# crisprVerse/screenCounter

Hardware: NVIDIA B200
Metric: reads/sec (higher is better)
Workload: dtype u32

## Files before the change

### screencounter_b200/csrc/jit.cpp

```cpp
#include "jit.hpp"

#include <dlfcn.h>
#include <sys/stat.h>
#include <sys/types.h>
#include <unistd.h>

#include <algorithm>
#include <cerrno>
#include <chrono>
#include <cstdio>

#include <cstdlib>
#include <cstring>
#include <map>
#include <mutex>
#include <sstream>
#include <vector>

#include "common.hpp"
#include "layout.hpp"

namespace scg {

namespace {
// ... 263 lines not shown
        if (rc != 0) {
            size_t log_size = 0;
            n.GetProgramLogSize(p, &log_size);
            std::string log(log_size, '\0');
            if (log_size) n.GetProgramLog(p, &log[0]);
            n.DestroyProgram(&p);
            return remember(std::string("nvrtcCompileProgram: ") + n.GetErrorString(rc) + "\n" + log);
        }
        size_t cubin_size = 0;
        n.GetCUBINSize(p, &cubin_size);
        cubin.resize(cubin_size);
        rc = n.GetCUBIN(p, cubin.data());
        n.DestroyProgram(&p);
        if (rc != 0 || cubin_size == 0) return remember("nvrtcGetCUBIN failed");
        if (!path.empty()) disk_store(path, disk_key, cubin);
    }
    if (const char* dump = std::getenv("SCG_DUMP_CUBIN")) {
        const std::string out = std::string(dump) + "/" + prog.name + ".cubin";
        if (FILE* f = std::fopen(out.c_str(), "wb")) {
            std::fwrite(cubin.data(), 1, cubin.size(), f);
            std::fclose(f);
        }
    }
    cudaError_t st = cudaLibraryLoadData(&entry.library, cubin.data(), nullptr, nullptr, 0, nullptr, nullptr, 0);
    if (st != cudaSuccess) {
        cudaGetLastError();
        return remember(std::string("cudaLibraryLoadData: ") + cudaGetErrorString(st));
    }
    for (const std::string& name : prog.kernels) {
        cudaKernel_t k = nullptr;
        st = cudaLibraryGetKernel(&k, entry.library, name.c_str());
        if (st != cudaSuccess) {
            cudaGetLastError();
            return remember("cudaLibraryGetKernel(" + name + "): " + cudaGetErrorString(st));
        }
        entry.kernels.push_back(k);
    }
    entry.build_s = wall_s() - t0;
    g_jit_seconds += entry.build_s;
    auto& slot = g_cache[key];
    slot = entry;
    return &slot;
}

double jit_seconds_total() { return g_jit_seconds; }

int jit_env_int(const char* name, int fallback, int lo, int hi) {
    const char* v = std::getenv(name);
    if (!v || !*v) return fallback;
    int x = std::atoi(v);
    return x < lo ? lo : (x > hi ? hi : x);
}

cudaKernel_t specialised_single_kernel(const SpecSingleConfig& cfg, int device, std::string* why, cudaKernel_t* slow) {
    auto fail = [&](const std::string& msg) -> cudaKernel_t {
        if (why) *why = msg;
        return nullptr;
    };
    if (cfg.W > (cfg.ulen > 0 ? 10 : 6)) {
        return fail(cfg.ulen > 0 ? "reads longer than 320 bases use the generic kernel" : "reads longer than 192 bases use the generic kernel");
    }
    if (cfg.T > 128) return fail("templates longer than 128 bases use the generic kernel");
    if (cfg.cb > 3) return fail("mismatch budgets above 7 use the generic kernel");
    if (cfg.keylen > 32) return fail("variable regions longer than 32 bases use the generic kernel");

    const int min_blocks = jit_env_int("SCG_SPEC_MIN_BLOCKS", cfg.ulen > 0 ? (cfg.W <= 3 ? 8 : (cfg.W <= 6 ? 6 : 4)) : 4, 1, 16);
    const int stages = jit_env_int("SCG_SPEC_STAGES", 2, 1, 8);
    const int group = jit_env_int("SCG_SPEC_GROUP", (cfg.ulen > 0 && cfg.W >= 6) ? 1 : 2, 1, 8);
    const int samples = jit_env_int("SCG_SPEC_SAMPLES", 8, 1, 32);

    std::string seed_list = "{ ";
    for (size_t k = 0; k < cfg.seed_masks.size(); ++k) seed_list += (k ? ", " : "") + std::to_string(cfg.seed_masks[k]) + "u";
    if (cfg.seed_masks.empty()) seed_list += "0u";
    seed_list += " }";
    std::ostringstream src;
    const int nb_max = (32 * cfg.W - cfg.T + 1 + 31) / 32;
    const int nb = std::max(1, std::min(cfg.nb, nb_max));
    src << "#define SPEC_CUSTOM 1\n"
        << "#define SPEC_T " << cfg.T << "\n"
        << "#define SPEC_FBASES \"" << cfg.fbases << "\"\n"
        << "#define SPEC_RBASES \"" << cfg.rbases << "\"\n"
        << "#define SPEC_FWD " << cfg.fwd << "\n"
        << "#define SPEC_REV " << cfg.rev << "\n"
        << "#define SPEC_W " << cfg.W << "\n"
        << "#define SPEC_NB " << nb << "\n"
        << "#define SPEC_CB " << cfg.cb << "\n"
        << "#define SPEC_MM " << cfg.mm << "\n"
        << "#define SPEC_MAXMM " << cfg.maxmm << "\n"
        << "#define SPEC_USE_FIRST " << cfg.use_first << "\n"
        << "#define SPEC_FSTART " << cfg.fstart << "\n"
        << "#define SPEC_RSTART " << cfg.rstart << "\n"
        << "#define SPEC_KEYLEN " << cfg.keylen << "\n"
        << "#define SPEC_NSEEDS " << cfg.seed_masks.size() << "\n"
        << "#define SPEC_SEEDMASKS " << seed_list << "\n"
        << "#define SPEC_DUP_FIRST " << cfg.dup_first << "\n"
        << "#define SPEC_NAME spec_single_kernel\n"
        << "#define SPEC_MIN_BLOCKS " << min_blocks << "\n"
        << "#define SPEC_STAGES " << stages << "\n"
        << "#define SPEC_ULEN " << cfg.ulen << "\n"
        << "#define SPEC_NAME_U spec_single_kernel_u\n"
        << "#define SPEC_NAME_SLOW spec_single_kernel_slow\n"
        << "#define SPEC_GROUP " << group << "\n"
        << "#define SPEC_SAMPLES " << samples << "\n"
        << "#define SPEC_INFO " << cfg.info << "\n"
        << "#define SPEC_JOINT " << cfg.joint << "\n"
        << "#define SPEC_HAS_INDEX " << cfg.has_index << "\n"
        << "#define SPEC_IBUCKETS " << cfg.ibuckets << "\n"
        << "#define SPEC_RAGGED " << cfg.ragged << "\n"
        << "#define SPEC_HIST " << cfg.hist << "\n"
        << "#define SPEC_PRED " << cfg.pred << "\n"
        << "#define SPEC_UWARP " << jit_env_int("SCG_SPEC_UWARP", 0, 0, 1) << "\n"
        << "#define SPEC_SKIP_GENERAL " << (cfg.ulen > 0 ? 1 : 0) << "\n"
        << "#include \"spec_single.cuh\"\n";
    JitProgram prog;
    prog.name = "spec_single_jit.cu";
    prog.text = src.str();
    if (cfg.ulen > 0) {
        prog.kernels = { "spec_single_kernel_u", "spec_single_kernel_slow" };
    } else {
        prog.kernels = { "spec_single_kernel" };
    }
    const JitModule* mod = jit_module(prog, device, why);
    if (!mod) return nullptr;
    if (slow) *slow = cfg.ulen > 0 ? mod->kernels[1] : nullptr;
    return mod->kernels[0];
}

}
```

### screencounter_b200/csrc/jit.hpp

```cpp
#pragma once

#include <cuda_runtime.h>

#include <string>
#include <vector>

#include "handlers_params.hpp"
#include "template_spec.hpp"

namespace scg {

struct SpecSingleConfig {
    std::string fbases, rbases;
    int T = 0, fwd = 0, rev = 0;
    int W = 0;
    int nb = 1;
    int cb = 0, mm = 0, maxmm = 0, use_first = 1;
    int fstart = 0, rstart = 0, keylen = 0;
    std::vector<uint32_t> seed_masks;
    int dup_first = 0;
    int ulen = 0;
    int info = 1;
    int joint = 0;
    int has_index = 1;
    int ibuckets = 0;
    int ragged = 0;
    int pred = 0;
    int hist = 0;
    std::string key() const;
};

struct JitProgram {
    std::string name;
    std::string text;
    std::vector<std::string> kernels;
};
struct JitModule {
    cudaLibrary_t library = nullptr;
    std::vector<cudaKernel_t> kernels;
    std::string problem;
    bool from_disk = false;
    double build_s = 0;
};
const JitModule* jit_module(const JitProgram& prog, int device, std::string* why);
double jit_seconds_total();
int jit_env_int(const char* name, int fallback, int lo, int hi);

cudaKernel_t specialised_single_kernel(const SpecSingleConfig& cfg, int device, std::string* why, cudaKernel_t* slow = nullptr);

int specialised_blocks_per_sm(cudaKernel_t kernel);

std::string jit_status();

}
```

### screencounter_b200/csrc/runners_single.cu

```cuda
#include <algorithm>
#include <chrono>
#include <cstring>
#include <exception>
#include <thread>

#include "api_common.hpp"
#include "hostpool.hpp"
#include "handlers.cuh"
#include "jit.hpp"
#include "launchers.hpp"
#include "matchers.hpp"

namespace scg {

std::string& creation_error() {
    static thread_local std::string msg;
    return msg;
}

static double now_s() {
    return std::chrono::duration<double>(std::chrono::steady_clock::now().time_since_epoch()).count();
}

Pool::Pool(const char* const* p, int n) {
// ... 284 lines not shown
    if (lib.KW != 1 || lib.nseeds < 1 || lib.nseeds > 4 || lib.cand_rows.empty()) return;
    for (int s = 0; s < lib.nseeds; ++s) {
        if (lib.seed_masks[s] == 0) {
            cfg.seed_masks.clear();
            return;
        }
        cfg.seed_masks.push_back(lib.seed_masks[s]);
    }
}

void launch_single(Context& ctx, const ReadsDev& reads, const SingleMatcher& m, int32_t* d_counts, int32_t* d_index, uint32_t* d_info,
                   cudaStream_t stream) {
    if (reads.n <= 0) return;
    const SingleParams& P = m.params;
    const long long ntiles = (reads.n + TILE - 1) / TILE;
    const int grid = ctx.grid_for(ntiles);

    SpecSingleConfig cfg;
    cfg.fbases = m.tmpl.fwd_seq;
    cfg.rbases = m.tmpl.rev ? m.tmpl.rev_seq : std::string(m.tmpl.length, '-');
    cfg.T = m.tmpl.length;
    cfg.fwd = m.tmpl.fwd ? 1 : 0;
    cfg.rev = m.tmpl.rev ? 1 : 0;
    cfg.W = reads.W;
    cfg.nb = std::max(1, (reads.uniform_len - m.tmpl.length + 1 + 31) / 32);
    cfg.cb = P.spec.cbits;
    cfg.mm = P.spec.mm;
    cfg.maxmm = P.max_mm;
    cfg.use_first = P.use_first;
    cfg.fstart = P.spec.fstart[0];
    cfg.rstart = P.spec.rstart[0];
    cfg.keylen = P.spec.rlen_f[0];
    spec_seeds(m, cfg);
    {
        const int nwin = reads.uniform_len - m.tmpl.length + 1;
        int nconst = 0;
        for (char ch : m.tmpl.fwd_seq) nconst += ch != '-';
        const bool want_u = !std::getenv("SCG_SPEC_NO_UNIFORM");
        if (want_u && nwin >= 1 && P.spec.mm >= 0 && P.spec.mm <= 3 && nconst >= 4 * (P.spec.mm + 1) &&
            cfg.T <= 128 && reads.W + 2 >= (cfg.T + 31) / 32 + 1 && reads.n <= 0x7FFFFFC0ll) {
            cfg.ulen = reads.uniform_len;
            cfg.ragged = reads.lens != nullptr ? 1 : 0;
            cfg.info = d_info ? 1 : 0;
            cfg.joint = (m.joint.ptr != nullptr && m.joint_shift != 0 && !std::getenv("SCG_SPEC_NO_JOINT")) ? 1 : 0;
            cfg.has_index = d_index ? 1 : 0;
            cfg.ibuckets = (m.have_ibuckets && !std::getenv("SCG_SPEC_NO_IBUCKETS")) ? 1 : 0;
            const int hist_max = jit_env_int("SCG_SPEC_HIST_MAX", 1024, 0, 8192);
            if (m.npool > 0 && m.npool <= hist_max) cfg.hist = (m.npool + 31) / 32 * 32;
            cfg.pred = jit_env_int("SCG_SPEC_PRED", 0, 0, 1);
        }
    }
    std::string why;
    cudaKernel_t slow = nullptr;
    cudaKernel_t spec = (P.spec.mm >= 0 && cfg.T > 0) ? specialised_single_kernel(cfg, ctx.device, &why, &slow) : nullptr;
    if (spec) {
        ReadsDev reads_arg = reads;
        SpecTables tables;
        std::memset(&tables, 0, sizeof tables);
        const DeviceLibrary* both[2] = { m.tmpl.fwd ? &m.lib_f : nullptr, m.tmpl.rev ? &m.lib_r : nullptr };
        for (int s = 0; s < 2; ++s) {
            if (!both[s]) continue;
            tables.slots[s] = reinterpret_cast<const uint4*>(both[s]->dev.slots);
            tables.buckets[s] = both[s]->dev.buckets;
            tables.cand_rows[s] = both[s]->dev.cand_rows;
            tables.slot_mask[s] = both[s]->dev.slot_mask;
            tables.bucket_mask[s] = both[s]->dev.bucket_mask;
            tables.nentries[s] = both[s]->dev.nentries;
        }
        tables.libs = P.libs;
        tables.joint = m.joint.as<uint4>();
        tables.ibuckets[0] = m.ibuckets[0].as<uint4>();
        tables.ibuckets[1] = m.ibuckets[1].as<uint4>();
        tables.joint_shift = m.joint_shift;
        const int resident = specialised_blocks_per_sm(spec);
        const int spec_grid = (int)std::max<long long>(1, std::min<long long>((ntiles + 3) / 4, (long long)ctx.sm_count * resident));
        if (cfg.ulen > 0) {
            ctx.slow_list.reserve((size_t)(ntiles * TILE) * sizeof(uint32_t));
            ctx.slow_count.reserve(sizeof(uint32_t));
            uint32_t* d_list = ctx.slow_list.as<uint32_t>();
            uint32_t* d_count = ctx.slow_count.as<uint32_t>();
            SCG_CUDA_CHECK(cudaMemsetAsync(d_count, 0, sizeof(uint32_t), stream));
            void* args[] = { &reads_arg, &tables, &d_counts, &d_index, &d_info, &d_list, &d_count };
            SCG_CUDA_CHECK(cudaLaunchKernel(reinterpret_cast<const void*>(spec), dim3(spec_grid), dim3(128), args, 0, stream));
            const LibDev* libs = P.libs;
            void* slow_args[] = { &reads_arg, &libs, &d_list, &d_count, &d_counts, &d_index, &d_info };
            const int slow_grid = (int)std::max<long long>(1, std::min<long long>((ntiles + 3) / 4, (long long)ctx.sm_count * 2));
            SCG_CUDA_CHECK(cudaLaunchKernel(reinterpret_cast<const void*>(slow), dim3(slow_grid), dim3(128), slow_args, 0, stream));
            ++ctx.launches;
        } else {
            void* args[] = { &reads_arg, &tables, &d_counts, &d_index, &d_info };
            SCG_CUDA_CHECK(cudaLaunchKernel(reinterpret_cast<const void*>(spec), dim3(spec_grid), dim3(128), args, 0, stream));
        }
        m.kernel_note = cfg.ulen > 0 ? std::string("specialised (NVRTC), ") + (cfg.ragged ? "trimmed reads, " : "uniform-length ") +
                                           "filter+verify, " + std::to_string(resident) + " blocks/SM"
                                     : "specialised (NVRTC)";
        ctx.kernel_note = m.kernel_note;
    } else {
        dispatch_cb(P.spec.cbits, [&](auto CB) {
            dispatch_kw(P.kw, [&](auto KW) {
                single_kernel<decltype(CB)::value, decltype(KW)::value><<<grid, 128, 0, stream>>>(reads, P, d_counts, d_index, d_info);
            });
        });
        m.kernel_note = "generic (" + why + ")";
        ctx.kernel_note = m.kernel_note;
    }
    SCG_CUDA_CHECK(cudaGetLastError());
    ++ctx.launches;
    ++ctx.timing.launches;
}

}

using namespace scg;

extern "C" {

const char* scg_version(void) { return "screencounter_b200 0.1.0 (sm_100a)"; }

int scg_ctx_create(scg_ctx** out, int device) {
    try {
        *out = new scg_ctx(device);
        return 0;
    } catch (const std::exception& e) {
        creation_error() = e.what();
        return 1;
    }
}

void scg_ctx_destroy(scg_ctx* ctx) { delete ctx; }

const char* scg_last_error(const scg_ctx* ctx) { return ctx ? ctx->impl.last_error.c_str() : creation_error().c_str(); }

const char* scg_timing_json(const scg_ctx* ctx) { return ctx ? ctx->impl.timing_json.c_str() : "{}"; }

long long scg_kernel_launches(const scg_ctx* ctx) {
    if (!ctx) return 0;
    long long n = ctx->impl.launches;
    for (const auto& p : ctx->peers) n += p->impl.launches;
    return n;
}

size_t scg_result_rows(const scg_result* r) { return r ? r->rows() : 0; }
int scg_result_width(const scg_result* r) { return r ? r->width : 0; }
size_t scg_result_reads(const scg_result* r) { return (r && r->trace_width) ? r->trace_index.size() / r->trace_width : 0; }
int scg_result_trace_width(const scg_result* r) { return r ? r->trace_width : 0; }

int scg_result_copy_table(const scg_result* r, int32_t* keys, char* strings, int32_t* freq) {
// ... 411 lines not shown
```

### screencounter_b200/csrc/spec_single.cuh

```cuda
#pragma once

#include "device_keys.cuh"

#ifndef SPEC_CUSTOM
#define SPEC_T 44
#define SPEC_FBASES "CAGCTACGTACG--------------------CCAGCTCGATCG"
#define SPEC_RBASES "CGATCGAGCTGG--------------------CGTACGTAGCTG"
#define SPEC_FWD 1
#define SPEC_REV 1
#define SPEC_W 3
#define SPEC_NB 2
#define SPEC_CB 1
#define SPEC_MM 1
#define SPEC_MAXMM 1
#define SPEC_USE_FIRST 1
#define SPEC_FSTART 12
#define SPEC_RSTART 12
#define SPEC_KEYLEN 20
#define SPEC_NAME spec_single_kernel_default
#endif

#ifndef SPEC_BLOCK
#define SPEC_BLOCK 128
#endif
#ifndef SPEC_MIN_BLOCKS
#define SPEC_MIN_BLOCKS 6
#endif
#ifndef SPEC_STAGES
#define SPEC_STAGES 2
#endif
#ifndef SPEC_NSEEDS
#define SPEC_NSEEDS 2
#define SPEC_SEEDMASKS { 0x3FFu, 0xFFC00u }
#endif
#ifndef SPEC_DUP_FIRST
#define SPEC_DUP_FIRST 0
#endif
#ifndef SPEC_ULEN
#ifdef SPEC_CUSTOM
#define SPEC_ULEN 0
#else
#define SPEC_ULEN 75
#endif
#endif
#ifndef SPEC_NAME_U
#define SPEC_NAME_U spec_single_kernel_u_default
#endif
#ifndef SPEC_NAME_SLOW
#define SPEC_NAME_SLOW spec_single_kernel_slow_default
#endif
#ifndef SPEC_GROUP
#define SPEC_GROUP 2
#endif
#ifndef SPEC_INFO
#define SPEC_INFO 1
#endif
#ifndef SPEC_JOINT
#define SPEC_JOINT 0
#endif
#ifndef SPEC_HAS_INDEX
#define SPEC_HAS_INDEX 1
#endif
#ifndef SPEC_IBUCKETS
#define SPEC_IBUCKETS 0
#endif
#ifndef SPEC_RAGGED
#define SPEC_RAGGED 0
#endif
#ifndef SPEC_PRED
#define SPEC_PRED 0
#endif
#ifndef SPEC_UWARP
#define SPEC_UWARP 0
#endif
#ifndef SPEC_HIST
#define SPEC_HIST 0
#endif

namespace scg {
namespace spec {

constexpr int T = SPEC_T;
constexpr int W = SPEC_W;
constexpr int NB = SPEC_NB;
constexpr int CB = SPEC_CB;
constexpr int KEYLEN = SPEC_KEYLEN;
constexpr int WARPS = SPEC_BLOCK / 32;
constexpr int QCAP = 64;
constexpr int STAGES = SPEC_STAGES;
constexpr int TILE_WORDS = 3 * W * TILE;
constexpr uint32_t TILE_BYTES = TILE_WORDS * 4u;
constexpr char FB[] = SPEC_FBASES;
constexpr char RB[] = SPEC_RBASES;

__host__ __device__ constexpr int count_constant(const char* s) {
    int n = 0;
    for (int j = 0; j < T; ++j) n += s[j] != '-';
    return n;
}
__host__ __device__ constexpr int kth_constant(const char* s, int k) {
    int n = 0;
    for (int j = 0; j < T; ++j) {
        if (s[j] != '-') {
            if (n == k) return j;
            ++n;
// ... 499 lines not shown
            waiting -= take;
            const bool active = lane < take;
            const uint32_t qi = active ? queue[0][waiting + lane] : 0u;
            const uint32_t qm = active ? queue[1][waiting + lane] : 0u;
            const uint32_t qh = active ? queue[2][waiting + lane] : 0u;
            const uint32_t ql = active ? queue[3][waiting + lane] : 0u;
            const uint32_t qn = active ? queue[4][waiting + lane] : 0u;
            __syncwarp();
            const bool simple = active && NSEEDS > 0 && !(qm & (PM_MANY | PM_LATE));
            if (NSEEDS > 0) {
                const bool rev = (qm & PM_REV) != 0;
                const int fc = (int)((qm >> 16) & 0xFFu);
                const Hit h = seeded_search(tb, rev, qh, ql, qn, SPEC_MAXMM - fc, simple);
                if (simple) {
                    const bool found = h.index >= 0;
                    if (found) atomicAdd(counts + h.index, 1);
                    if (out_index) out_index[qi] = h.index;
                    if (out_info) out_info[qi] = pack_info(found, rev, fc + h.dist, h.dist, (int)(qm & 0xFFFFu));
                }
            }
            if (__any_sync(0xFFFFFFFFu, active && !simple)) {
                slow_single(reads, tb.libs, (long long)qi, active && !simple, counts, out_index, out_info);
            }
        }
        if (!have) break;
        tile += nwarps;
    }
}
#endif


#if SPEC_ULEN > 0

namespace scg {
namespace spec {

constexpr int ULEN = SPEC_ULEN;
constexpr int NWIN = ULEN - T + 1;
static_assert(NWIN >= 1, "the uniform-length kernel needs reads at least as long as the template");
constexpr int NBLOCKS = (NWIN + 31) / 32;
template <int PB>
__host__ __device__ constexpr uint32_t block_mask() {
    return NWIN - 32 * PB >= 32 ? 0xFFFFFFFFu : ((1u << (NWIN - 32 * PB)) - 1u);
}
constexpr int TW = (T + 31) / 32;
constexpr int GROUP = SPEC_GROUP;
constexpr int NGROUPS = SPEC_MM + 1;
#ifndef SPEC_SAMPLES
#define SPEC_SAMPLES 8
#endif
constexpr int SAMPLES = SPEC_SAMPLES;
static_assert(W + 2 >= TW + 1, "window words plus their funnel partner must exist");
static_assert(NBLOCKS - 1 + TW <= W, "the last block's window words and their funnel partners lie within the guarded words");

template <bool REV, int G>
struct Group {
    static constexpr int NC = REV ? NCR : NCF;
    static constexpr int lo = NC * G / NGROUPS, hi = NC * (G + 1) / NGROUPS, size = hi - lo;
    static constexpr int S = size < SAMPLES ? size : SAMPLES;
    __host__ __device__ static constexpr int sample(int k) { return lo + (S > 0 ? k * size / S : 0); }
};

template <bool REV, int PB, int G, int K>
__device__ __forceinline__ uint32_t group_any(const Planes& P) {
    using Gr = Group<REV, G>;
    if constexpr (K >= Gr::S) {
        return 0u;
    } else if constexpr (K + 3 <= Gr::S) {
        return cplane<REV, Gr::sample(K)>(P, PB) | cplane<REV, Gr::sample(K + 1)>(P, PB) |
               cplane<REV, Gr::sample(K + 2)>(P, PB) | group_any<REV, PB, G, K + 3>(P);
    } else if constexpr (K + 2 <= Gr::S) {
        return cplane<REV, Gr::sample(K)>(P, PB) | cplane<REV, Gr::sample(K + 1)>(P, PB) | group_any<REV, PB, G, K + 2>(P);
    } else {
        return cplane<REV, Gr::sample(K)>(P, PB) | group_any<REV, PB, G, K + 1>(P);
    }
}

template <bool REV, int PB, int G>
__device__ __forceinline__ uint32_t all_groups_dirty(const Planes& P) {
    if constexpr (G >= NGROUPS) {
        return 0xFFFFFFFFu;
    } else if constexpr (Group<REV, G>::S == 0) {
        return 0u;
    } else {
        return group_any<REV, PB, G, 0>(P) & all_groups_dirty<REV, PB, G + 1>(P);
    }
}

template <bool REV, int PB>
__device__ __forceinline__ uint32_t candidate_windows(const Planes& P, uint32_t live) {
    return ~all_groups_dirty<REV, PB, 0>(P) & live;
}

__host__ __device__ constexpr uint32_t template_word(const char* s, int k, int what) {
    uint32_t w = 0;
    for (int j = 0; j < 32; ++j) {
        const int pos = 32 * k + j;
        if (pos >= T || s[pos] == '-') continue;
        const char c = s[pos];
        const uint32_t code = (c == 'A' || c == 'a') ? 0u : ((c == 'C' || c == 'c') ? 1u : ((c == 'G' || c == 'g') ? 2u : 3u));
        const uint32_t bit = what == 0 ? 1u : (what == 1 ? (code >> 1) : (code & 1u));
        w |= bit << j;
    }
    return w;
}

template <int K, int PB>
__device__ __forceinline__ int verify_words(const Words& R, int p, bool rev, uint32_t (&wh)[TW + 1], uint32_t (&wl)[TW + 1],
                                            uint32_t (&wn)[TW + 1]) {
    if constexpr (K >= TW) {
        return 0;
    } else {
        constexpr uint32_t fth = template_word(FB, K, 1), ftl = template_word(FB, K, 2), fcm = template_word(FB, K, 0);
        constexpr uint32_t rth = template_word(RB, K, 1), rtl = template_word(RB, K, 2), rcm = template_word(RB, K, 0);
        wh[K] = __funnelshift_r(R.h[PB + K], R.h[PB + K + 1], p);
        wl[K] = __funnelshift_r(R.l[PB + K], R.l[PB + K + 1], p);
        wn[K] = __funnelshift_r(R.n[PB + K], R.n[PB + K + 1], p);
        const uint32_t th = (SPEC_FWD && SPEC_REV) ? (rev ? rth : fth) : (SPEC_REV ? rth : fth);
        const uint32_t tl = (SPEC_FWD && SPEC_REV) ? (rev ? rtl : ftl) : (SPEC_REV ? rtl : ftl);
        const uint32_t cm = (SPEC_FWD && SPEC_REV) ? (rev ? rcm : fcm) : (SPEC_REV ? rcm : fcm);
        return __popc(((wh[K] ^ th) | (wl[K] ^ tl) | wn[K]) & cm) + verify_words<K + 1, PB>(R, p, rev, wh, wl, wn);
    }
}
template <int PB>
__device__ __forceinline__ int verify_window(const Words& R, int p, bool rev, uint32_t (&wh)[TW + 1], uint32_t (&wl)[TW + 1],
                                             uint32_t (&wn)[TW + 1]) {
    wh[TW] = wl[TW] = wn[TW] = 0;
    return verify_words<0, PB>(R, p, rev, wh, wl, wn);
}

template <int START>
__device__ __forceinline__ uint32_t window_key(const uint32_t (&w)[TW + 1]) {
    constexpr int a = START >> 5, sh = START & 31;
    const uint32_t lo = w[a], hi = a + 1 <= TW ? w[a + 1] : 0u;
    return (sh == 0 ? lo : __funnelshift_r(lo, hi, sh)) & KEYMASK;
}

template <int PB>
__device__ __forceinline__ void scan_blocks(const Words& R, const Planes& P, int npos, int& ncand, uint32_t& meta, uint32_t& kh,
                                            uint32_t& kl, uint32_t& kn) {
    if constexpr (PB < NBLOCKS) {
#if SPEC_RAGGED
        const int left = npos - 32 * PB;
        const uint32_t live = left <= 0 ? 0u : (left >= 32 ? 0xFFFFFFFFu : ((1u << left) - 1u));
#else
        const uint32_t live = npos > 0 ? block_mask<PB>() : 0u;
#endif
        uint32_t cf = SPEC_FWD ? candidate_windows<false, PB>(P, live) : 0u;
        uint32_t cr = SPEC_REV ? candidate_windows<true, PB>(P, live) : 0u;
        bool more = PB == 0 ? true : __any_sync(0xFFFFFFFFu, (cf | cr) != 0u);
        while (more) {
            const uint32_t any = cf | cr;
            const uint32_t lowest = any & (0u - any);
            const int p = 31 - __clz(lowest | 1u);
            const bool rev = SPEC_FWD ? !(cf & lowest) : true;
            if (rev) {
                cr &= ~lowest;
            } else {
                cf &= ~lowest;
            }
            uint32_t wh[TW + 1], wl[TW + 1], wn[TW + 1];
            const int c = verify_window<PB>(R, p, rev, wh, wl, wn);
            const bool ok = lowest != 0u && c <= SPEC_MM;
            if (ok && ncand == 0) {
                meta = PM_CAND + (rev ? PM_REV : 0u) + ((uint32_t)c << 16) + (uint32_t)(32 * PB + p);
                if (SPEC_FSTART == SPEC_RSTART || !SPEC_REV || !SPEC_FWD) {
                    constexpr int START = (SPEC_FWD && SPEC_REV) ? SPEC_FSTART : (SPEC_FWD ? SPEC_FSTART : SPEC_RSTART);
                    kh = window_key<START>(wh);
                    kl = window_key<START>(wl);
                    kn = window_key<START>(wn);
                } else {
                    kh = rev ? window_key<SPEC_RSTART>(wh) : window_key<SPEC_FSTART>(wh);
                    kl = rev ? window_key<SPEC_RSTART>(wl) : window_key<SPEC_FSTART>(wl);
                    kn = rev ? window_key<SPEC_RSTART>(wn) : window_key<SPEC_FSTART>(wn);
                }
            }
            ncand += ok ? 1 : 0;
            more = __any_sync(0xFFFFFFFFu, (cf | cr) != 0u);
        }
        scan_blocks<PB + 1>(R, P, npos, ncand, meta, kh, kl, kn);
    }
}

__device__ __forceinline__ void drain_deferred(const SpecTables& tb, const uint32_t (*queue)[QCAP], int at, int take, int lane,
                                               int32_t* __restrict__ counts, uint32_t hist_saddr, int32_t* __restrict__ out_index,
                                               uint32_t* __restrict__ out_info, uint32_t* __restrict__ slow_list,
                                               uint32_t* __restrict__ slow_count) {
    const bool active = lane < take;
    const uint32_t qi = active ? queue[0][at + lane] : 0u;
    const uint32_t qm = active ? queue[1][at + lane] : 0u;
    const uint32_t qh = active ? queue[2][at + lane] : 0u;
    const uint32_t ql = active ? queue[3][at + lane] : 0u;
    const uint32_t qn = active ? queue[4][at + lane] : 0u;
    __syncwarp();
    const bool simple = active && NSEEDS > 0 && !(qm & PM_MANY);
    if (NSEEDS > 0) {
        const bool rev = (qm & PM_REV) != 0;
        const int fc = (int)((qm >> 16) & 0xFFu);
        const Hit h = seeded_search(tb, rev, qh, ql, qn, SPEC_MAXMM - fc, simple);
        if (simple) {
            const bool found = h.index >= 0;
            if (found) count_hit(counts, hist_saddr, h.index);
            if (out_index) out_index[qi] = h.index;
            if (SPEC_INFO && out_info) out_info[qi] = pack_info(found, rev, fc + h.dist, h.dist, (int)(qm & 0xFFFFu));
        }
    }
    const uint32_t hard = __ballot_sync(0xFFFFFFFFu, active && !simple);
    if (hard) {
        const int leader = __ffs(hard) - 1;
        uint32_t base = 0;
        if (lane == leader) base = atomicAdd(slow_count, (uint32_t)__popc(hard));
        base = __shfl_sync(0xFFFFFFFFu, base, leader);
        if (active && !simple) slow_list[base + __popc(hard & ((1u << lane) - 1u))] = qi;
    }
}

}
}

extern "C" __global__ void __launch_bounds__(SPEC_BLOCK, SPEC_MIN_BLOCKS)
    SPEC_NAME_U(const scg::ReadsDev reads, const scg::SpecTables tb, int32_t* __restrict__ counts, int32_t* __restrict__ out_index,
                uint32_t* __restrict__ out_info, uint32_t* __restrict__ slow_list, uint32_t* __restrict__ slow_count) {
    using namespace scg;
    using namespace scg::spec;
    static_assert(KEYLEN <= 32, "the specialised kernel handles variable regions of at most 32 bases");
    constexpr uint32_t GROUP_BYTES = GROUP * TILE_BYTES;
    __shared__ __align__(128) uint32_t stage_all[WARPS][STAGES][GROUP * TILE_WORDS];
    __shared__ __align__(8) unsigned long long bar_all[WARPS][STAGES];
    __shared__ uint32_t queue_all[WARPS][5][QCAP];
#if SPEC_HIST
    __shared__ int32_t hist[SPEC_HIST];
    for (int k = threadIdx.x; k < SPEC_HIST; k += SPEC_BLOCK) hist[k] = 0;
    __syncthreads();
    const uint32_t hist_saddr = smem_addr(hist);
#else
    const uint32_t hist_saddr = 0;
#endif
#if SPEC_UWARP
    const int wib = __shfl_sync(0xFFFFFFFFu, (int)(threadIdx.x >> 5), 0);
#else
    const int wib = threadIdx.x >> 5;
#endif
    uint32_t(*queue)[QCAP] = queue_all[wib];
    int waiting = 0;

    const int lane = threadIdx.x & 31;
    const uint32_t lanes_below = (1u << lane) - 1u;
#if SPEC_UWARP
    const int warp = (int)(blockIdx.x * (blockDim.x >> 5)) + wib;
#else
    const int warp = (int)((blockIdx.x * blockDim.x + threadIdx.x) >> 5);
#endif
    const int nwarps = (int)((gridDim.x * blockDim.x) >> 5);
    const uint32_t n = (uint32_t)reads.n;
    const int ntiles = (int)((n + TILE - 1) / TILE);
    const int ngroups = (ntiles + GROUP - 1) / GROUP;

    const uint32_t stage_base = smem_addr(&stage_all[wib][0][0]);
    const uint32_t bar_base = smem_addr(&bar_all[wib][0]);
    if (lane == 0) {
#pragma unroll
        for (int s = 0; s < STAGES; ++s) mbar_init(bar_base + 8u * s, 1);
        fence_barrier_init();
    }
    __syncwarp();
    uint64_t stream_policy;
    asm volatile("createpolicy.fractional.L2::evict_first.b64 %0, 1.0;" : "=l"(stream_policy));
    auto fetch = [&](int g, uint32_t stage) {
        const int tiles = min(GROUP, ntiles - GROUP * g);
        const uint32_t bytes = (uint32_t)tiles * TILE_BYTES;
        const uint32_t bar = bar_base + 8u * stage;
        const char* src = reinterpret_cast<const char*>(reads.data) + (size_t)g * GROUP_BYTES;
        asm volatile(
            "{\n\t.reg .pred p;\n\t"
            "elect.sync _|p, 0xFFFFFFFF;\n\t"
            "@p mbarrier.arrive.expect_tx.shared::cta.b64 _, [%0], %1;\n\t"
            "@p cp.async.bulk.shared::cluster.global.mbarrier::complete_tx::bytes.L2::cache_hint [%2], [%3], %1, [%0], %4;\n\t}"
            ::"r"(bar), "r"(bytes), "r"(stage_base + stage * GROUP_BYTES), "l"(src), "l"(stream_policy)
            : "memory");
    };
#pragma unroll
    for (int s = 0; s < STAGES; ++s) {
        if (warp + s * nwarps < ngroups) fetch(warp + s * nwarps, (uint32_t)s);
    }

    constexpr uint32_t PU_MISS_DEFERS = 1u << 25, PU_ALWAYS_DEFERS = 1u << 24;
    Pending pend;
    pend.meta = 0;
    pend.a = pend.b = make_uint4(0, 0, 0, 0);
    pend.kh = pend.kl = pend.i = 0;
    uint32_t stage = 0, parity = 0;
    int group = warp;
    int tile_in_group = 0, tiles_here = 0;
    bool have = group < ngroups;
    if (have) {
        mbar_wait(bar_base, 0);
        tiles_here = min(GROUP, ntiles - GROUP * group);
    }
    for (;;) {
        uint32_t meta = 0, kh = 0, kl = 0, kn = 0, i = 0;
        if (have) {
            Words R;
            const uint32_t* buf = stage_all[wib][stage] + tile_in_group * TILE_WORDS + lane;
#pragma unroll
            for (int w = 0; w < W; ++w) {
                R.h[w] = buf[(PLANE_H * W + w) * TILE];
                R.l[w] = buf[(PLANE_L * W + w) * TILE];
                R.n[w] = buf[(PLANE_N * W + w) * TILE];
            }
            R.h[W] = R.l[W] = R.n[W] = 0;
            R.h[W + 1] = R.l[W + 1] = R.n[W + 1] = 0;
            i = (uint32_t)(group * GROUP + tile_in_group) * TILE + lane;
            const bool inrange = i < n;
            Planes P;
            make_planes(R, P);

#if SPEC_RAGGED
            const int npos = inrange ? (int)reads.lens[i] - T + 1 : 0;
#else
            const int npos = inrange ? NWIN : 0;
#endif
            int ncand = 0;
            scan_blocks<0>(R, P, npos, ncand, meta, kh, kl, kn);
            {
                const bool many = ncand > 1;
                const int fc = (int)((meta >> 16) & 0xFFu);
                const bool cand = (meta & PM_CAND) != 0;
                const bool miss_defers = cand && ((SPEC_MAXMM - fc >= 1) || many);
                const bool always_defers = cand && many && !SPEC_USE_FIRST;
                meta += (inrange ? PM_INRANGE : 0u) + (many ? PM_MANY : 0u) + (miss_defers ? PU_MISS_DEFERS : 0u) +
                        (always_defers ? PU_ALWAYS_DEFERS : 0u);
            }

            if (++tile_in_group == tiles_here) {
                __syncwarp();
                const int ahead = group + STAGES * nwarps;
                if (ahead < ngroups) fetch(ahead, stage);
            }
        }

        {
            const uint32_t m = pend.meta;
            int index = -1;
            if (m & PM_PROBED) {
                const int ra = (pend.a.x == pend.kh && pend.a.y == pend.kl) ? (int)pend.a.z : -1;
                const int rb = (pend.b.x == pend.kh && pend.b.y == pend.kl) ? (int)pend.b.z : -1;
                index = max(ra, rb);
            }
            const bool defer = (m & PU_ALWAYS_DEFERS) || ((m & PU_MISS_DEFERS) && index < 0);
#if SPEC_PRED && !SPEC_HIST && !SPEC_INFO
            {
                const bool settled = (m & PM_INRANGE) && !defer;
                pred_red_add1(counts + max(index, 0), settled && index >= 0);
                if (SPEC_HAS_INDEX) pred_stcs(out_index + pend.i, index, settled);
            }
#else
            if ((m & PM_INRANGE) && !defer) {
                if (index >= 0) count_hit(counts, hist_saddr, index);
                if (SPEC_HAS_INDEX) __stcs(out_index + pend.i, index);
                if (SPEC_INFO && out_info) {
                    __stcs(out_info + pend.i, pack_info(index >= 0, (m & PM_REV) != 0, (int)((m >> 16) & 0xFFu), 0, (int)(m & 0xFFFFu)));
                }
            }
#endif
            const uint32_t dm = __ballot_sync(0xFFFFFFFFu, defer);
            if (dm) {
                if (defer) {
                    const int at = waiting + __popc(dm & lanes_below);
                    queue[0][at] = pend.i;
                    queue[1][at] = m;
#if SPEC_JOINT
                    queue[2][at] = pend.kh & 0x7FFFFFFFu;
#else
                    queue[2][at] = pend.kh;
#endif
                    queue[3][at] = pend.kl;
                    queue[4][at] = (m & PM_PROBED) ? 0u : pend.a.x;
                }
                waiting += __popc(dm);
                __syncwarp();
            }
        }

        pend.meta = meta;
        pend.i = i;
        pend.kl = kl;
        pend.a.x = kn;
#if SPEC_JOINT
        pend.kh = kh + ((meta & PM_REV) ? 0x80000000u : 0u);
#if SPEC_PRED
        {
            const bool probe = (meta & PM_CAND) && kn == 0;
            const uint32_t x = joint_hash(pend.kh, kl);
            const uint32_t second = (1u << (32 - tb.joint_shift)) + (joint_hash2(x) >> tb.joint_shift);
            pred_ldcg(pend.a, tb.joint + (x >> tb.joint_shift), probe);
            pred_ldcg(pend.b, tb.joint + second, probe);
            pend.meta = meta + (probe ? PM_PROBED : 0u);
        }
#else
        if ((meta & PM_CAND) && kn == 0) {
            const uint32_t x = joint_hash(pend.kh, kl);
            const uint32_t second = (1u << (32 - tb.joint_shift)) + (joint_hash2(x) >> tb.joint_shift);
            pend.a = __ldcg(tb.joint + (x >> tb.joint_shift));
            pend.b = __ldcg(tb.joint + second);
            pend.meta = meta + PM_PROBED;
        }
#endif
#else
        pend.kh = kh;
        if ((meta & PM_CAND) && kn == 0) {
            const bool frev = (meta & PM_REV) != 0;
            const uint4* __restrict__ slots = frev ? tb.slots[1] : tb.slots[0];
            const uint32_t mask = frev ? tb.slot_mask[1] : tb.slot_mask[0];
            const uint32_t acc = hash_key(&kh, &kl, 1, 0);
            pend.a = __ldcg(slots + (acc & mask));
            pend.b = __ldcg(slots + (size_t)(mask + 1) + (hash_second(acc) & mask));
            pend.meta = meta + PM_PROBED;
        }
#endif

        while (waiting >= 32 || (!have && waiting > 0)) {
            const int take = waiting < 32 ? waiting : 32;
            waiting -= take;
            drain_deferred(tb, queue, waiting, take, lane, counts, hist_saddr, out_index, out_info, slow_list, slow_count);
        }
        if (!have) break;
        if (tile_in_group == tiles_here) {
            group += nwarps;
            tile_in_group = 0;
            if (++stage == STAGES) {
                stage = 0;
                parity ^= 1u;
            }
            have = group < ngroups;
            if (have) {
                mbar_wait(bar_base + 8u * stage, parity);
                tiles_here = min(GROUP, ntiles - GROUP * group);
            }
        }
    }
#if SPEC_HIST
    __syncthreads();
    for (int k = threadIdx.x; k < SPEC_HIST; k += SPEC_BLOCK) {
        const int32_t v = hist[k];
        if (v) atomicAdd(counts + k, v);
    }
#endif
}

extern "C" __global__ void __launch_bounds__(128)
    SPEC_NAME_SLOW(const scg::ReadsDev reads, const scg::LibDev* __restrict__ libs, const uint32_t* __restrict__ slow_list,
                   const uint32_t* __restrict__ slow_count, int32_t* __restrict__ counts, int32_t* __restrict__ out_index,
                   uint32_t* __restrict__ out_info) {
    using namespace scg;
    using namespace scg::spec;
    const uint32_t total = *slow_count;
    const uint32_t stride = gridDim.x * blockDim.x;
    for (uint32_t base = (blockIdx.x * blockDim.x + threadIdx.x) & ~31u; base < total; base += stride) {
        const uint32_t k = base + (threadIdx.x & 31);
        const bool active = k < total;
        const uint32_t i = active ? slow_list[k] : 0u;
        slow_single(reads, libs, (long long)i, active, counts, out_index, out_info);
    }
}

#endif
```

Baseline: 66.98 billion.

## Process two tiles per iteration in the uniform-length specialised kernel

Adds a pair mode to the JIT specialised kernel: each warp filters both tiles of a group, then verifies their candidates in a shared loop, and settles and issues hash-table probes for two pending reads per iteration. This aims to raise instruction-level parallelism and hide probe latency by keeping two independent lookups in flight per lane. In exchange it uses more registers, so the minimum-blocks launch bound is lowered, and the per-warp deferral queue grows to 96 entries. Mode is on by default for uniform reads with group size 2 and W>=4.

```diff
diff --git a/screencounter_b200/csrc/jit.cpp b/screencounter_b200/csrc/jit.cpp
--- a/screencounter_b200/csrc/jit.cpp
+++ b/screencounter_b200/csrc/jit.cpp
@@ -339,7 +339,7 @@
     return x < lo ? lo : (x > hi ? hi : x);
 }
 
-cudaKernel_t specialised_single_kernel(const SpecSingleConfig& cfg, int device, std::string* why, cudaKernel_t* slow) {
+cudaKernel_t specialised_single_kernel(const SpecSingleConfig& cfg, int device, std::string* why, cudaKernel_t* slow, bool* pair) {
     auto fail = [&](const std::string& msg) -> cudaKernel_t {
         if (why) *why = msg;
         return nullptr;
@@ -351,10 +351,12 @@
     if (cfg.cb > 3) return fail("mismatch budgets above 7 use the generic kernel");
     if (cfg.keylen > 32) return fail("variable regions longer than 32 bases use the generic kernel");
 
-    const int min_blocks = jit_env_int("SCG_SPEC_MIN_BLOCKS", cfg.ulen > 0 ? (cfg.W <= 3 ? 8 : (cfg.W <= 6 ? 6 : 4)) : 4, 1, 16);
     const int stages = jit_env_int("SCG_SPEC_STAGES", 2, 1, 8);
     const int group = jit_env_int("SCG_SPEC_GROUP", (cfg.ulen > 0 && cfg.W >= 6) ? 1 : 2, 1, 8);
     const int samples = jit_env_int("SCG_SPEC_SAMPLES", 8, 1, 32);
+    const int use_pair = (cfg.ulen > 0 && group == 2) ? jit_env_int("SCG_SPEC_PAIR", cfg.W >= 4 ? 1 : 0, 0, 1) : 0;
+    const int min_blocks = jit_env_int("SCG_SPEC_MIN_BLOCKS",
+                                       cfg.ulen > 0 ? (use_pair ? (cfg.W <= 4 ? 6 : 5) : (cfg.W <= 3 ? 8 : (cfg.W <= 6 ? 6 : 4))) : 4, 1, 16);
 
     std::string seed_list = "{ ";
     for (size_t k = 0; k < cfg.seed_masks.size(); ++k) seed_list += (k ? ", " : "") + std::to_string(cfg.seed_masks[k]) + "u";
@@ -388,6 +390,7 @@
         << "#define SPEC_NAME_U spec_single_kernel_u\n"
         << "#define SPEC_NAME_SLOW spec_single_kernel_slow\n"
         << "#define SPEC_GROUP " << group << "\n"
+        << "#define SPEC_PAIR " << use_pair << "\n"
         << "#define SPEC_SAMPLES " << samples << "\n"
         << "#define SPEC_INFO " << cfg.info << "\n"
         << "#define SPEC_JOINT " << cfg.joint << "\n"
@@ -410,6 +413,7 @@
     const JitModule* mod = jit_module(prog, device, why);
     if (!mod) return nullptr;
     if (slow) *slow = cfg.ulen > 0 ? mod->kernels[1] : nullptr;
+    if (pair) *pair = use_pair != 0;
     return mod->kernels[0];
 }
 
diff --git a/screencounter_b200/csrc/jit.hpp b/screencounter_b200/csrc/jit.hpp
--- a/screencounter_b200/csrc/jit.hpp
+++ b/screencounter_b200/csrc/jit.hpp
@@ -46,7 +46,8 @@
 double jit_seconds_total();
 int jit_env_int(const char* name, int fallback, int lo, int hi);
 
-cudaKernel_t specialised_single_kernel(const SpecSingleConfig& cfg, int device, std::string* why, cudaKernel_t* slow = nullptr);
+cudaKernel_t specialised_single_kernel(const SpecSingleConfig& cfg, int device, std::string* why, cudaKernel_t* slow = nullptr,
+                                       bool* pair = nullptr);
 
 int specialised_blocks_per_sm(cudaKernel_t kernel);
 
diff --git a/screencounter_b200/csrc/runners_single.cu b/screencounter_b200/csrc/runners_single.cu
--- a/screencounter_b200/csrc/runners_single.cu
+++ b/screencounter_b200/csrc/runners_single.cu
@@ -360,7 +360,8 @@
     }
     std::string why;
     cudaKernel_t slow = nullptr;
-    cudaKernel_t spec = (P.spec.mm >= 0 && cfg.T > 0) ? specialised_single_kernel(cfg, ctx.device, &why, &slow) : nullptr;
+    bool pair = false;
+    cudaKernel_t spec = (P.spec.mm >= 0 && cfg.T > 0) ? specialised_single_kernel(cfg, ctx.device, &why, &slow, &pair) : nullptr;
     if (spec) {
         ReadsDev reads_arg = reads;
         SpecTables tables;
@@ -400,7 +401,8 @@
             SCG_CUDA_CHECK(cudaLaunchKernel(reinterpret_cast<const void*>(spec), dim3(spec_grid), dim3(128), args, 0, stream));
         }
         m.kernel_note = cfg.ulen > 0 ? std::string("specialised (NVRTC), ") + (cfg.ragged ? "trimmed reads, " : "uniform-length ") +
-                                           "filter+verify, " + std::to_string(resident) + " blocks/SM"
+                                           "filter+verify, " + (pair ? "two tiles per iteration (spec_single_kernel_u+pair), " : "") +
+                                           std::to_string(resident) + " blocks/SM"
                                      : "specialised (NVRTC)";
         ctx.kernel_note = m.kernel_note;
     } else {
diff --git a/screencounter_b200/csrc/spec_single.cuh b/screencounter_b200/csrc/spec_single.cuh
--- a/screencounter_b200/csrc/spec_single.cuh
+++ b/screencounter_b200/csrc/spec_single.cuh
@@ -51,6 +51,9 @@
 #endif
 #ifndef SPEC_GROUP
 #define SPEC_GROUP 2
+#endif
+#ifndef SPEC_PAIR
+#define SPEC_PAIR 0
 #endif
 #ifndef SPEC_INFO
 #define SPEC_INFO 1
@@ -656,6 +659,9 @@
 constexpr int SAMPLES = SPEC_SAMPLES;
 static_assert(W + 2 >= TW + 1, "window words plus their funnel partner must exist");
 static_assert(NBLOCKS - 1 + TW <= W, "the last block's window words and their funnel partners lie within the guarded words");
+constexpr bool PAIR = SPEC_PAIR != 0;
+static_assert(!PAIR || GROUP == 2, "the pair loop consumes groups of exactly two tiles");
+constexpr int UQCAP = PAIR ? 96 : 64;
 
 template <bool REV, int G>
 struct Group {
@@ -740,53 +746,192 @@
     return (sh == 0 ? lo : __funnelshift_r(lo, hi, sh)) & KEYMASK;
 }
 
+struct Scan {
+    int ncand;
+    uint32_t meta, kh, kl, kn;
+};
+
 template <int PB>
-__device__ __forceinline__ void scan_blocks(const Words& R, const Planes& P, int npos, int& ncand, uint32_t& meta, uint32_t& kh,
-                                            uint32_t& kl, uint32_t& kn) {
+__device__ __forceinline__ void block_candidates(const Planes& P, int npos, uint32_t& cf, uint32_t& cr) {
+#if SPEC_RAGGED
+    const int left = npos - 32 * PB;
+    const uint32_t live = left <= 0 ? 0u : (left >= 32 ? 0xFFFFFFFFu : ((1u << left) - 1u));
+#else
+    const uint32_t live = npos > 0 ? block_mask<PB>() : 0u;
+#endif
+    cf = SPEC_FWD ? candidate_windows<false, PB>(P, live) : 0u;
+    cr = SPEC_REV ? candidate_windows<true, PB>(P, live) : 0u;
+}
+
+template <int PB>
+__device__ __forceinline__ void verify_next(const Words& R, uint32_t& cf, uint32_t& cr, Scan& s) {
+    const uint32_t any = cf | cr;
+    const uint32_t lowest = any & (0u - any);
+    const int p = 31 - __clz(lowest | 1u);
+    const bool rev = SPEC_FWD ? !(cf & lowest) : true;
+    if (rev) {
+        cr &= ~lowest;
+    } else {
+        cf &= ~lowest;
+    }
+    uint32_t wh[TW + 1], wl[TW + 1], wn[TW + 1];
+    const int c = verify_window<PB>(R, p, rev, wh, wl, wn);
+    const bool ok = lowest != 0u && c <= SPEC_MM;
+    if (ok && s.ncand == 0) {
+        s.meta = PM_CAND + (rev ? PM_REV : 0u) + ((uint32_t)c << 16) + (uint32_t)(32 * PB + p);
+        if (SPEC_FSTART == SPEC_RSTART || !SPEC_REV || !SPEC_FWD) {
+            constexpr int START = (SPEC_FWD && SPEC_REV) ? SPEC_FSTART : (SPEC_FWD ? SPEC_FSTART : SPEC_RSTART);
+            s.kh = window_key<START>(wh);
+            s.kl = window_key<START>(wl);
+            s.kn = window_key<START>(wn);
+        } else {
+            s.kh = rev ? window_key<SPEC_RSTART>(wh) : window_key<SPEC_FSTART>(wh);
+            s.kl = rev ? window_key<SPEC_RSTART>(wl) : window_key<SPEC_FSTART>(wl);
+            s.kn = rev ? window_key<SPEC_RSTART>(wn) : window_key<SPEC_FSTART>(wn);
+        }
+    }
+    s.ncand += ok ? 1 : 0;
+}
+
+template <int PB>
+__device__ __forceinline__ void scan_blocks(const Words& R, const Planes& P, int npos, Scan& s) {
     if constexpr (PB < NBLOCKS) {
-#if SPEC_RAGGED
-        const int left = npos - 32 * PB;
-        const uint32_t live = left <= 0 ? 0u : (left >= 32 ? 0xFFFFFFFFu : ((1u << left) - 1u));
-#else
-        const uint32_t live = npos > 0 ? block_mask<PB>() : 0u;
-#endif
-        uint32_t cf = SPEC_FWD ? candidate_windows<false, PB>(P, live) : 0u;
-        uint32_t cr = SPEC_REV ? candidate_windows<true, PB>(P, live) : 0u;
+        uint32_t cf, cr;
+        block_candidates<PB>(P, npos, cf, cr);
         bool more = PB == 0 ? true : __any_sync(0xFFFFFFFFu, (cf | cr) != 0u);
         while (more) {
-            const uint32_t any = cf | cr;
-            const uint32_t lowest = any & (0u - any);
-            const int p = 31 - __clz(lowest | 1u);
-            const bool rev = SPEC_FWD ? !(cf & lowest) : true;
-            if (rev) {
-                cr &= ~lowest;
-            } else {
-                cf &= ~lowest;
-            }
-            uint32_t wh[TW + 1], wl[TW + 1], wn[TW + 1];
-            const int c = verify_window<PB>(R, p, rev, wh, wl, wn);
-            const bool ok = lowest != 0u && c <= SPEC_MM;
-            if (ok && ncand == 0) {
-                meta = PM_CAND + (rev ? PM_REV : 0u) + ((uint32_t)c << 16) + (uint32_t)(32 * PB + p);
-                if (SPEC_FSTART == SPEC_RSTART || !SPEC_REV || !SPEC_FWD) {
-                    constexpr int START = (SPEC_FWD && SPEC_REV) ? SPEC_FSTART : (SPEC_FWD ? SPEC_FSTART : SPEC_RSTART);
-                    kh = window_key<START>(wh);
-                    kl = window_key<START>(wl);
-                    kn = window_key<START>(wn);
-                } else {
-                    kh = rev ? window_key<SPEC_RSTART>(wh) : window_key<SPEC_FSTART>(wh);
-                    kl = rev ? window_key<SPEC_RSTART>(wl) : window_key<SPEC_FSTART>(wl);
-                    kn = rev ? window_key<SPEC_RSTART>(wn) : window_key<SPEC_FSTART>(wn);
-                }
-            }
-            ncand += ok ? 1 : 0;
+            verify_next<PB>(R, cf, cr, s);
             more = __any_sync(0xFFFFFFFFu, (cf | cr) != 0u);
         }
-        scan_blocks<PB + 1>(R, P, npos, ncand, meta, kh, kl, kn);
-    }
-}
-
-__device__ __forceinline__ void drain_deferred(const SpecTables& tb, const uint32_t (*queue)[QCAP], int at, int take, int lane,
+        scan_blocks<PB + 1>(R, P, npos, s);
+    }
+}
+
+template <int PB>
+__device__ __forceinline__ void filter_blocks(const Planes& P, int npos, uint32_t (&cf)[NBLOCKS], uint32_t (&cr)[NBLOCKS]) {
+    if constexpr (PB < NBLOCKS) {
+        block_candidates<PB>(P, npos, cf[PB], cr[PB]);
+        filter_blocks<PB + 1>(P, npos, cf, cr);
+    }
+}
+
+template <int PB>
+__device__ __forceinline__ void verify_blocks_pair(const Words& RA, uint32_t (&cfA)[NBLOCKS], uint32_t (&crA)[NBLOCKS], Scan& A,
+                                                   const Words& RB, uint32_t (&cfB)[NBLOCKS], uint32_t (&crB)[NBLOCKS], Scan& B) {
+    if constexpr (PB < NBLOCKS) {
+        bool more = PB == 0 ? true : __any_sync(0xFFFFFFFFu, (cfA[PB] | crA[PB] | cfB[PB] | crB[PB]) != 0u);
+        while (more) {
+            verify_next<PB>(RA, cfA[PB], crA[PB], A);
+            verify_next<PB>(RB, cfB[PB], crB[PB], B);
+            more = __any_sync(0xFFFFFFFFu, (cfA[PB] | crA[PB] | cfB[PB] | crB[PB]) != 0u);
+        }
+        verify_blocks_pair<PB + 1>(RA, cfA, crA, A, RB, cfB, crB, B);
+    }
+}
+
+__device__ __forceinline__ void load_words(const uint32_t* buf, Words& R) {
+#pragma unroll
+    for (int w = 0; w < W; ++w) {
+        R.h[w] = buf[(PLANE_H * W + w) * TILE];
+        R.l[w] = buf[(PLANE_L * W + w) * TILE];
+        R.n[w] = buf[(PLANE_N * W + w) * TILE];
+    }
+    R.h[W] = R.l[W] = R.n[W] = 0;
+    R.h[W + 1] = R.l[W + 1] = R.n[W + 1] = 0;
+}
+
+constexpr uint32_t PU_MISS_DEFERS = 1u << 25, PU_ALWAYS_DEFERS = 1u << 24;
+
+__device__ __forceinline__ uint32_t settle_flags(const Scan& s, bool inrange) {
+    const bool many = s.ncand > 1;
+    const int fc = (int)((s.meta >> 16) & 0xFFu);
+    const bool cand = (s.meta & PM_CAND) != 0;
+    const bool miss_defers = cand && ((SPEC_MAXMM - fc >= 1) || many);
+    const bool always_defers = cand && many && !SPEC_USE_FIRST;
+    return s.meta + (inrange ? PM_INRANGE : 0u) + (many ? PM_MANY : 0u) + (miss_defers ? PU_MISS_DEFERS : 0u) +
+           (always_defers ? PU_ALWAYS_DEFERS : 0u);
+}
+
+__device__ __forceinline__ bool settle(const Pending& pend, int32_t* __restrict__ counts, uint32_t hist_saddr, int32_t* __restrict__ out_index,
+                                       uint32_t* __restrict__ out_info) {
+    const uint32_t m = pend.meta;
+    int index = -1;
+    if (m & PM_PROBED) {
+        const int ra = (pend.a.x == pend.kh && pend.a.y == pend.kl) ? (int)pend.a.z : -1;
+        const int rb = (pend.b.x == pend.kh && pend.b.y == pend.kl) ? (int)pend.b.z : -1;
+        index = max(ra, rb);
+    }
+    const bool defer = (m & PU_ALWAYS_DEFERS) || ((m & PU_MISS_DEFERS) && index < 0);
+#if SPEC_PRED && !SPEC_HIST && !SPEC_INFO
+    {
+        const bool settled = (m & PM_INRANGE) && !defer;
+        pred_red_add1(counts + max(index, 0), settled && index >= 0);
+        if (SPEC_HAS_INDEX) pred_stcs(out_index + pend.i, index, settled);
+    }
+#else
+    if ((m & PM_INRANGE) && !defer) {
+        if (index >= 0) count_hit(counts, hist_saddr, index);
+        if (SPEC_HAS_INDEX) __stcs(out_index + pend.i, index);
+        if (SPEC_INFO && out_info) {
+            __stcs(out_info + pend.i, pack_info(index >= 0, (m & PM_REV) != 0, (int)((m >> 16) & 0xFFu), 0, (int)(m & 0xFFFFu)));
+        }
+    }
+#endif
+    return defer;
+}
+
+__device__ __forceinline__ void enqueue(uint32_t (*queue)[UQCAP], int at, const Pending& pend) {
+    queue[0][at] = pend.i;
+    queue[1][at] = pend.meta;
+#if SPEC_JOINT
+    queue[2][at] = pend.kh & 0x7FFFFFFFu;
+#else
+    queue[2][at] = pend.kh;
+#endif
+    queue[3][at] = pend.kl;
+    queue[4][at] = (pend.meta & PM_PROBED) ? 0u : pend.a.x;
+}
+
+__device__ __forceinline__ void request(Pending& pend, const SpecTables& tb, uint32_t meta, uint32_t i, uint32_t kh, uint32_t kl, uint32_t kn) {
+    pend.meta = meta;
+    pend.i = i;
+    pend.kl = kl;
+    pend.a.x = kn;
+#if SPEC_JOINT
+    pend.kh = kh + ((meta & PM_REV) ? 0x80000000u : 0u);
+#if SPEC_PRED
+    {
+        const bool probe = (meta & PM_CAND) && kn == 0;
+        const uint32_t x = joint_hash(pend.kh, kl);
+        const uint32_t second = (1u << (32 - tb.joint_shift)) + (joint_hash2(x) >> tb.joint_shift);
+        pred_ldcg(pend.a, tb.joint + (x >> tb.joint_shift), probe);
+        pred_ldcg(pend.b, tb.joint + second, probe);
+        pend.meta = meta + (probe ? PM_PROBED : 0u);
+    }
+#else
+    if ((meta & PM_CAND) && kn == 0) {
+        const uint32_t x = joint_hash(pend.kh, kl);
+        const uint32_t second = (1u << (32 - tb.joint_shift)) + (joint_hash2(x) >> tb.joint_shift);
+        pend.a = __ldcg(tb.joint + (x >> tb.joint_shift));
+        pend.b = __ldcg(tb.joint + second);
+        pend.meta = meta + PM_PROBED;
+    }
+#endif
+#else
+    pend.kh = kh;
+    if ((meta & PM_CAND) && kn == 0) {
+        const bool frev = (meta & PM_REV) != 0;
+        const uint4* __restrict__ slots = frev ? tb.slots[1] : tb.slots[0];
+        const uint32_t mask = frev ? tb.slot_mask[1] : tb.slot_mask[0];
+        const uint32_t acc = hash_key(&kh, &kl, 1, 0);
+        pend.a = __ldcg(slots + (acc & mask));
+        pend.b = __ldcg(slots + (size_t)(mask + 1) + (hash_second(acc) & mask));
+        pend.meta = meta + PM_PROBED;
+    }
+#endif
+}
+
+__device__ __forceinline__ void drain_deferred(const SpecTables& tb, const uint32_t (*queue)[UQCAP], int at, int take, int lane,
                                                int32_t* __restrict__ counts, uint32_t hist_saddr, int32_t* __restrict__ out_index,
                                                uint32_t* __restrict__ out_info, uint32_t* __restrict__ slow_list,
                                                uint32_t* __restrict__ slow_count) {
@@ -831,7 +976,7 @@
     constexpr uint32_t GROUP_BYTES = GROUP * TILE_BYTES;
     __shared__ __align__(128) uint32_t stage_all[WARPS][STAGES][GROUP * TILE_WORDS];
     __shared__ __align__(8) unsigned long long bar_all[WARPS][STAGES];
-    __shared__ uint32_t queue_all[WARPS][5][QCAP];
+    __shared__ uint32_t queue_all[WARPS][5][UQCAP];
 #if SPEC_HIST
     __shared__ int32_t hist[SPEC_HIST];
     for (int k = threadIdx.x; k < SPEC_HIST; k += SPEC_BLOCK) hist[k] = 0;
@@ -845,7 +990,7 @@
 #else
     const int wib = threadIdx.x >> 5;
 #endif
-    uint32_t(*queue)[QCAP] = queue_all[wib];
+    uint32_t(*queue)[UQCAP] = queue_all[wib];
     int waiting = 0;
 
     const int lane = threadIdx.x & 31;
@@ -888,13 +1033,81 @@
         if (warp + s * nwarps < ngroups) fetch(warp + s * nwarps, (uint32_t)s);
     }
 
-    constexpr uint32_t PU_MISS_DEFERS = 1u << 25, PU_ALWAYS_DEFERS = 1u << 24;
     Pending pend;
     pend.meta = 0;
     pend.a = pend.b = make_uint4(0, 0, 0, 0);
     pend.kh = pend.kl = pend.i = 0;
     uint32_t stage = 0, parity = 0;
     int group = warp;
+#if SPEC_PAIR
+    Pending pend2 = pend;
+    for (;;) {
+        const bool have = group < ngroups;
+        Scan A{ 0, 0, 0, 0, 0 }, B{ 0, 0, 0, 0, 0 };
+        uint32_t metaA = 0, metaB = 0;
+        const uint32_t iA = (uint32_t)group * (GROUP * TILE) + lane, iB = iA + TILE;
+        if (have) {
+            mbar_wait(bar_base + 8u * stage, parity);
+            const uint32_t* buf = stage_all[wib][stage] + lane;
+            Words RA, RB;
+            load_words(buf, RA);
+            load_words(buf + TILE_WORDS, RB);
+            const bool inA = iA < n, inB = iB < n;
+#if SPEC_RAGGED
+            const int nposA = inA ? (int)reads.lens[iA] - T + 1 : 0;
+            const int nposB = inB ? (int)reads.lens[iB] - T + 1 : 0;
+#else
+            const int nposA = inA ? NWIN : 0;
+            const int nposB = inB ? NWIN : 0;
+#endif
+            uint32_t cfA[NBLOCKS], crA[NBLOCKS], cfB[NBLOCKS], crB[NBLOCKS];
+            {
+                Planes P;
+                make_planes(RA, P);
+                filter_blocks<0>(P, nposA, cfA, crA);
+            }
+            {
+                Planes P;
+                make_planes(RB, P);
+                filter_blocks<0>(P, nposB, cfB, crB);
+            }
+            verify_blocks_pair<0>(RA, cfA, crA, A, RB, cfB, crB, B);
+            metaA = settle_flags(A, inA);
+            metaB = settle_flags(B, inB);
+
+            __syncwarp();
+            const int ahead = group + STAGES * nwarps;
+            if (ahead < ngroups) fetch(ahead, stage);
+            if (++stage == STAGES) {
+                stage = 0;
+                parity ^= 1u;
+            }
+        }
+
+        {
+            const bool dA = settle(pend, counts, hist_saddr, out_index, out_info);
+            const bool dB = settle(pend2, counts, hist_saddr, out_index, out_info);
+            const uint32_t dmA = __ballot_sync(0xFFFFFFFFu, dA), dmB = __ballot_sync(0xFFFFFFFFu, dB);
+            if (dmA | dmB) {
+                if (dA) enqueue(queue, waiting + __popc(dmA & lanes_below), pend);
+                if (dB) enqueue(queue, waiting + __popc(dmA) + __popc(dmB & lanes_below), pend2);
+                waiting += __popc(dmA) + __popc(dmB);
+                __syncwarp();
+            }
+        }
+
+        request(pend, tb, metaA, iA, A.kh, A.kl, A.kn);
+        request(pend2, tb, metaB, iB, B.kh, B.kl, B.kn);
+
+        while (waiting >= 32 || (!have && waiting > 0)) {
+            const int take = waiting < 32 ? waiting : 32;
+            waiting -= take;
+            drain_deferred(tb, queue, waiting, take, lane, counts, hist_saddr, out_index, out_info, slow_list, slow_count);
+        }
+        if (!have) break;
+        group += nwarps;
+    }
+#else
     int tile_in_group = 0, tiles_here = 0;
     bool have = group < ngroups;
     if (have) {
@@ -902,18 +1115,11 @@
         tiles_here = min(GROUP, ntiles - GROUP * group);
     }
     for (;;) {
-        uint32_t meta = 0, kh = 0, kl = 0, kn = 0, i = 0;
+        Scan s{ 0, 0, 0, 0, 0 };
+        uint32_t meta = 0, i = 0;
         if (have) {
             Words R;
-            const uint32_t* buf = stage_all[wib][stage] + tile_in_group * TILE_WORDS + lane;
-#pragma unroll
-            for (int w = 0; w < W; ++w) {
-                R.h[w] = buf[(PLANE_H * W + w) * TILE];
-                R.l[w] = buf[(PLANE_L * W + w) * TILE];
-                R.n[w] = buf[(PLANE_N * W + w) * TILE];
-            }
-            R.h[W] = R.l[W] = R.n[W] = 0;
-            R.h[W + 1] = R.l[W + 1] = R.n[W + 1] = 0;
+            load_words(stage_all[wib][stage] + tile_in_group * TILE_WORDS + lane, R);
             i = (uint32_t)(group * GROUP + tile_in_group) * TILE + lane;
             const bool inrange = i < n;
             Planes P;
@@ -924,17 +1130,8 @@
 #else
             const int npos = inrange ? NWIN : 0;
 #endif
-            int ncand = 0;
-            scan_blocks<0>(R, P, npos, ncand, meta, kh, kl, kn);
-            {
-                const bool many = ncand > 1;
-                const int fc = (int)((meta >> 16) & 0xFFu);
-                const bool cand = (meta & PM_CAND) != 0;
-                const bool miss_defers = cand && ((SPEC_MAXMM - fc >= 1) || many);
-                const bool always_defers = cand && many && !SPEC_USE_FIRST;
-                meta += (inrange ? PM_INRANGE : 0u) + (many ? PM_MANY : 0u) + (miss_defers ? PU_MISS_DEFERS : 0u) +
-                        (always_defers ? PU_ALWAYS_DEFERS : 0u);
-            }
+            scan_blocks<0>(R, P, npos, s);
+            meta = settle_flags(s, inrange);
 
             if (++tile_in_group == tiles_here) {
                 __syncwarp();
@@ -944,84 +1141,16 @@
         }
 
         {
-            const uint32_t m = pend.meta;
-            int index = -1;
-            if (m & PM_PROBED) {
-                const int ra = (pend.a.x == pend.kh && pend.a.y == pend.kl) ? (int)pend.a.z : -1;
-                const int rb = (pend.b.x == pend.kh && pend.b.y == pend.kl) ? (int)pend.b.z : -1;
-                index = max(ra, rb);
-            }
-            const bool defer = (m & PU_ALWAYS_DEFERS) || ((m & PU_MISS_DEFERS) && index < 0);
-#if SPEC_PRED && !SPEC_HIST && !SPEC_INFO
-            {
-                const bool settled = (m & PM_INRANGE) && !defer;
-                pred_red_add1(counts + max(index, 0), settled && index >= 0);
-                if (SPEC_HAS_INDEX) pred_stcs(out_index + pend.i, index, settled);
-            }
-#else
-            if ((m & PM_INRANGE) && !defer) {
-                if (index >= 0) count_hit(counts, hist_saddr, index);
-                if (SPEC_HAS_INDEX) __stcs(out_index + pend.i, index);
-                if (SPEC_INFO && out_info) {
-                    __stcs(out_info + pend.i, pack_info(index >= 0, (m & PM_REV) != 0, (int)((m >> 16) & 0xFFu), 0, (int)(m & 0xFFFFu)));
-                }
-            }
-#endif
+            const bool defer = settle(pend, counts, hist_saddr, out_index, out_info);
             const uint32_t dm = __ballot_sync(0xFFFFFFFFu, defer);
             if (dm) {
-                if (defer) {
-                    const int at = waiting + __popc(dm & lanes_below);
-                    queue[0][at] = pend.i;
-                    queue[1][at] = m;
-#if SPEC_JOINT
-                    queue[2][at] = pend.kh & 0x7FFFFFFFu;
-#else
-                    queue[2][at] = pend.kh;
-#endif
-                    queue[3][at] = pend.kl;
-                    queue[4][at] = (m & PM_PROBED) ? 0u : pend.a.x;
-                }
+                if (defer) enqueue(queue, waiting + __popc(dm & lanes_below), pend);
                 waiting += __popc(dm);
                 __syncwarp();
             }
         }
 
-        pend.meta = meta;
-        pend.i = i;
-        pend.kl = kl;
-        pend.a.x = kn;
-#if SPEC_JOINT
-        pend.kh = kh + ((meta & PM_REV) ? 0x80000000u : 0u);
-#if SPEC_PRED
-        {
-            const bool probe = (meta & PM_CAND) && kn == 0;
-            const uint32_t x = joint_hash(pend.kh, kl);
-            const uint32_t second = (1u << (32 - tb.joint_shift)) + (joint_hash2(x) >> tb.joint_shift);
-            pred_ldcg(pend.a, tb.joint + (x >> tb.joint_shift), probe);
-            pred_ldcg(pend.b, tb.joint + second, probe);
-            pend.meta = meta + (probe ? PM_PROBED : 0u);
-        }
-#else
-        if ((meta & PM_CAND) && kn == 0) {
-            const uint32_t x = joint_hash(pend.kh, kl);
-            const uint32_t second = (1u << (32 - tb.joint_shift)) + (joint_hash2(x) >> tb.joint_shift);
-            pend.a = __ldcg(tb.joint + (x >> tb.joint_shift));
-            pend.b = __ldcg(tb.joint + second);
-            pend.meta = meta + PM_PROBED;
-        }
-#endif
-#else
-        pend.kh = kh;
-        if ((meta & PM_CAND) && kn == 0) {
-            const bool frev = (meta & PM_REV) != 0;
-            const uint4* __restrict__ slots = frev ? tb.slots[1] : tb.slots[0];
-            const uint32_t mask = frev ? tb.slot_mask[1] : tb.slot_mask[0];
-            const uint32_t acc = hash_key(&kh, &kl, 1, 0);
-            pend.a = __ldcg(slots + (acc & mask));
-            pend.b = __ldcg(slots + (size_t)(mask + 1) + (hash_second(acc) & mask));
-            pend.meta = meta + PM_PROBED;
-        }
-#endif
+        request(pend, tb, meta, i, s.kh, s.kl, s.kn);
 
         while (waiting >= 32 || (!have && waiting > 0)) {
             const int take = waiting < 32 ? waiting : 32;
@@ -1043,6 +1172,7 @@
             }
         }
     }
+#endif
 #if SPEC_HIST
     __syncthreads();
     for (int k = threadIdx.x; k < SPEC_HIST; k += SPEC_BLOCK) {
```

Result: faster. 67.91 billion (median of 6 runs) (+1.4%).
